# GuildOfWeavers/genSTARK

Measured on AMD Instinct MI355X. Metric: prove() ms + NTT GF(p) elements/sec, MiMC-128 2^20 steps, higher is better.
Workload: dtype u128; 1 GPU; MiMC-128 prove(), 2^20 steps, extensionFactor 16, exeQueryCount 48, friQueryCount 64, blake2s256; one independent proof per GPU; evaluation_domain=16777216, ntt_points_per_prove=17827072, ntt_transforms_per_prove=4, proof_bytes=371695

## Files before the change

genstark_amd/_abi.py:

```python
import ctypes as C
import os

_HERE = os.path.dirname(os.path.abspath(__file__))
HIP_LIB_PATH = os.path.join(_HERE, 'csrc', 'libgstark_hip.so')
MODULUS_128 = 2**128 - 9 * 2**32 + 1
MODULUS_64 = 2**64 - 21 * 2**30 + 1
MODULUS_32 = 2**32 - 3 * 2**25 + 1
MODULUS_17 = 96769
MODULUS_256 = 2**256 - 351 * 2**32 + 1
MODULUS_224 = 2**224 - 2**96 + 1
HIP_LIB_PATHS = {MODULUS_128: HIP_LIB_PATH, MODULUS_64: os.path.join(_HERE, 'csrc', 'libgstark_hip_q64.so'),
                 MODULUS_32: os.path.join(_HERE, 'csrc', 'libgstark_hip_q32.so'),
                 MODULUS_17: os.path.join(_HERE, 'csrc', 'libgstark_hip_q17.so'),
                 MODULUS_256: os.path.join(_HERE, 'csrc', 'libgstark_hip_p256.so'),
                 MODULUS_224: os.path.join(_HERE, 'csrc', 'libgstark_hip_p224.so')}
HIP_LIB_PATH_RUNTIME = os.path.join(_HERE, 'csrc', 'libgstark_hip_rt.so')

GS_OK = 0


class FriLayer(C.Structure):
    _fields_ = [('next', C.c_void_p), ('leaves', C.c_void_p), ('nodes', C.c_void_p), ('point_out', C.c_void_p), ('ticket', C.c_uint64)]

HASH_ALGS = {'sha256': 0, 'blake2s256': 1}
# ... 73 lines not shown
    'gs_small_interpolate': (_int, [_bytes, _bytes, _u32, _vp]),
    'gs_small_eval_poly': (_int, [_bytes, _u32, _bytes, _u32, _vp]),
    'gs_mimc_trace': (_int, [_vp, _bytes, _bytes, _u32, _u64, _vp]),
    'gs_mimc_constraints': (_int, [_vp, _vp, _u64, _u64, _vp, _u64, _vp]),
    'gs_mimc_composition': (_int, [_vp, _vp, _u64, _u64, _bytes, _vp, _u64, _bytes, _u64, _u64, _bytes, C.POINTER(_u64), _u32, _bytes, _vp]),
    'gs_pseudorandom_indexes': (_int, [_bytes, _u32, _u32, _u64, _u32, C.POINTER(_u64)]),
    'gs_air_trace_segments': (_int, [_vp, C.POINTER(_u32), _u32, C.POINTER(_u32), _u32, _bytes, _u32, _u32, _u32, _bytes, C.POINTER(_u32), _u32, _bytes, _u64, _u64, _vp]),
    'gs_air_trace': (_int, [_vp, C.POINTER(_u32), _u32, _bytes, _u32, _u32, _u32, _bytes, C.POINTER(_u32), _u32, _bytes, _u64, _vp]),
    'gs_air_constraints': (_int, [_vp, C.POINTER(_u32), _u32, _bytes, _u32, _u32, _u32, _u32, _vp, _u64, _u64, _vp,
                                  C.POINTER(_u64), _u32, _vp]),
    'gs_composition_tail': (_int, [_vp, _u64, _bytes, _vp, _vp, _u64, _bytes, _vp, _u32, _bytes, _u32, C.POINTER(_u64), C.POINTER(_u32), _u32, _bytes, _bytes,
                                   _vp, _u32, _bytes, _bytes, _vp, _u64, _vp, _vp]),
    'gs_composition_tail_coset': (_int, [_vp, _u64, _bytes, _bytes, _vp, _vp, _u64, _bytes, _vp, _u32, _bytes, _u32, C.POINTER(_u64), C.POINTER(_u32), _u32, _bytes,
                                         _bytes, _vp, _u32, _bytes, _bytes, _vp, _u64, _vp, _vp]),
    'gs_air_constraints_strided': (_int, [_vp, C.POINTER(_u32), _u32, _bytes, _u32, _u32, _u32, _u32, _vp, _u64, _u64, _u64, _u64, _vp,
                                          C.POINTER(_u64), _u32, _vp]),
}

EXPORTED_SYMBOLS = tuple(_SIGNATURES)

_OPTIONAL_SIGNATURES = {
    'gs_boundary_polys': (_int, [_vp, _bytes, _u64, _u64, C.POINTER(_u64), _bytes, C.POINTER(_u32), _u32, _u32, _vp, _vp]),
    'gs_boundary_schoolbook_log2': (_u32, [_u32]),
    'gs_eval_polys_at_points': (_int, [_vp, _vp, _u32, _u64, C.POINTER(_u64), _bytes, _u32, _vp]),
    'gs_eval_polys_at_points_segment': (_u32, []),
}
OPTIONAL_SYMBOLS = tuple(_OPTIONAL_SIGNATURES)

_HADES_SIGNATURES = {
    'gs_hades_create': (_int, [_vp, _u32, _u32, _u32, _u64, _bytes, _bytes, _pvp]),
    'gs_hades_destroy': (_int, [_vp, _vp]),
    'gs_hades_hash': (_int, [_vp, _vp, _vp, _u64, _u32, _u32, _vp]),
    'gs_hades_merkle': (_int, [_vp, _vp, _vp, _u64, _u32, _vp]),
    'gs_hades_merkle_paths': (_int, [_vp, _vp, _u64, _u32, C.POINTER(_u64), _u64, _vp]),
    'gs_hades_merkle_top': (_u32, []),
}
HADES_SYMBOLS = tuple(_HADES_SIGNATURES)

_RESCUE_SIGNATURES = {
    'gs_rescue_create': (_int, [_vp, _u32, _u32, _u64, _bytes, _bytes, _bytes, _pvp]),
    'gs_rescue_destroy': (_int, [_vp, _vp]),
    'gs_rescue_hash': (_int, [_vp, _vp, _vp, _u64, _u32, _u32, _u32, _u32, _vp]),
    'gs_rescue_merkle': (_int, [_vp, _vp, _vp, _u64, _vp]),
    'gs_rescue_spread_limit': (_u64, []),
}
RESCUE_SYMBOLS = tuple(_RESCUE_SIGNATURES)

_TREE_UPDATE_SIGNATURES = {
    'gs_hades_merkle_update': (_int, [_vp, _vp, _vp, _u64, _u32, C.POINTER(_u64), _vp, _u64, _vp, _vp]),
    'gs_rescue_merkle_update': (_int, [_vp, _vp, _vp, _u64, C.POINTER(_u64), _vp, _u64, _vp, _vp]),
}
TREE_UPDATE_SYMBOLS = tuple(_TREE_UPDATE_SIGNATURES)


class GstarkError(RuntimeError):
    pass


def load_library(path):
    if not os.path.exists(path):
        raise GstarkError(
            f'{path} not found: the HIP backend is not built (run `python -c "import __graft_entry__ as g; g.build()"`).'
            ' There is no CPU fallback.')
    lib = C.CDLL(path)
    for name, (res, args) in _SIGNATURES.items():
        fn = getattr(lib, name)
        fn.restype, fn.argtypes = res, args
    for name, (res, args) in (list(_OPTIONAL_SIGNATURES.items()) + list(_HADES_SIGNATURES.items()) + list(_RESCUE_SIGNATURES.items())
                              + list(_TREE_UPDATE_SIGNATURES.items())):
        fn = getattr(lib, name, None)
        if fn is not None:
            fn.restype, fn.argtypes = res, args
    return lib


class Backend:

    def __init__(self, device=0, stream=None, lib_path=None, allow_test_double=False, modulus=None):
        if lib_path is None:
            lib_path = HIP_LIB_PATH if modulus is None else HIP_LIB_PATHS.get(modulus, HIP_LIB_PATH_RUNTIME)
        self.lib = load_library(lib_path)
        self.element_size = self.lib.gs_element_size()
        if modulus is not None:
            if modulus < 3 or modulus >> (8 * self.element_size):
                raise GstarkError(f'a modulus of {modulus.bit_length()} bits does not fit {lib_path}')
            rc = self.lib.gs_set_modulus(modulus.to_bytes(self.element_size, 'little'), self.element_size)
            if rc != GS_OK:
                raise GstarkError(f'{lib_path} does not compute modulo {modulus} (gs_set_modulus: {rc}'
                                  + (': the runtime-modulus library serves ONE modulus per process, and it has been given another' if rc == -3 else '') + ')')
        buf = C.create_string_buffer(self.element_size)
        self.lib.gs_field_modulus(C.cast(buf, C.c_void_p))
        self.modulus = int.from_bytes(buf.raw, 'little')
        if modulus is not None and self.modulus != modulus:
            raise GstarkError(f'{lib_path} is built for the field of {self.modulus} elements, not {modulus}')
        if not self.modulus:
            raise GstarkError(f'{lib_path} takes its modulus at run time: pass modulus=')
        self.name = self.lib.gs_backend_name().decode()
        if self.name != 'hip-gfx950' and not allow_test_double:
            raise GstarkError(f'refusing backend {self.name!r}: the product path runs on hip-gfx950 only')
        if self.lib.gs_abi_version() != 1:
            raise GstarkError('gstark ABI version mismatch')
        ctx = C.c_void_p()
        rc = self.lib.gs_ctx_create(int(device), C.c_void_p(stream), C.byref(ctx))
        if rc != GS_OK or not ctx.value:
            raise GstarkError(f'gs_ctx_create(device={device}) failed with {rc}: no gfx950 device? (no CPU fallback)')
        self.ctx = ctx
        self.device = device
        self.stats = {}

    def jit(self, enable=True):
        self.call('gs_air_jit', 2 if enable == 'auto' else (1 if enable else 0))
        return self

    @property
    def jit_launches(self):
        return self.lib.gs_air_jit_launches(self.ctx)

    def traffic(self, on=None):
        if on is not None:
            self.call('gs_traffic_enable', 1 if on else 0)
            return self

# ... 66 lines not shown
```

genstark_amd/csrc/air_mimc.hip:

```cpp
#include "common.h"
#include "host_field.h"

__global__ void k_mimc_constraints(const fe *__restrict__ p, uint64_t nc, uint64_t shift, const fe *__restrict__ k, uint64_t klen,
                                   fe *__restrict__ out) {
    for (uint64_t j = blockIdx.x * (uint64_t)blockDim.x + threadIdx.x; j < nc; j += (uint64_t)gridDim.x * blockDim.x) {
        uint64_t jn = j + shift;
        if (jn >= nc) jn -= nc;
        fe x = p[j], nx = p[jn];
        fe x3 = fe_mul(fe_mul(x, x), x);
        out[j] = fe_sub(nx, fe_add(x3, k[j % klen]));
    }
}

#define GS_MIMC_COMP_MAX_PERIOD 32
#define GS_MIMC_COMP_MAX_ROOTS 4
struct MimcCompArgs {
    fe qz[GS_MIMC_COMP_MAX_PERIOD];
    fe bt[GS_MIMC_COMP_MAX_PERIOD];
    fe lt[GS_MIMC_COMP_MAX_PERIOD];
    fe ipoly[GS_MIMC_COMP_MAX_ROOTS];
    uint64_t root[GS_MIMC_COMP_MAX_ROOTS];
    fe x_last;
};
__global__ void k_mimc_composition(const fe *__restrict__ p, uint64_t n, uint64_t shift, const fe *__restrict__ k, uint64_t klen,
                                   const fe *__restrict__ tw_lo, const fe *__restrict__ tw_hi, int log_lo, int logn, const fe *__restrict__ u,
                                   MimcCompArgs a, uint32_t period, uint32_t nroots, int with_lc, fe *__restrict__ out) {
    __shared__ fe qz[GS_MIMC_COMP_MAX_PERIOD], bt[GS_MIMC_COMP_MAX_PERIOD], lt[GS_MIMC_COMP_MAX_PERIOD];
    if (threadIdx.x < period) { qz[threadIdx.x] = a.qz[threadIdx.x]; bt[threadIdx.x] = a.bt[threadIdx.x]; lt[threadIdx.x] = a.lt[threadIdx.x]; }
    __syncthreads();
    for (uint64_t i = blockIdx.x * (uint64_t)blockDim.x + threadIdx.x; i < n; i += (uint64_t)gridDim.x * blockDim.x) {
        fe x = tw_lo[i & ((1ull << log_lo) - 1)];
        if (logn > log_lo) x = fe_mul(x, tw_hi[i >> log_lo]);
        const fe pi = p[i], pn = p[(i + shift) & (n - 1)];
        const fe q = fe_sub(pn, fe_add(fe_mul(fe_mul(pi, pi), pi), k[i % klen]));
        const fe d = fe_mul(fe_mul(q, fe_sub(x, a.x_last)), qz[i & (period - 1)]);
        fe iv = a.ipoly[nroots - 1];
        for (int c = (int)nroots - 2; c >= 0; c--) iv = fe_add(fe_mul(iv, x), a.ipoly[c]);
        fe b = fe_mul(fe_sub(pi, iv), bt[i & (period - 1)]);
        for (uint32_t r = 0; r < nroots; r++) b = fe_mul(b, u[(i + n - a.root[r]) & (n - 1)]);
        fe r = fe_add(d, b);
        if (with_lc) r = fe_add(r, fe_mul(pi, lt[i & (period - 1)]));
        out[i] = r;
    }
}

#define GS_MIMC_CHUNK_BODY(STEP)                                                                                \
    for (uint64_t i = base; i < end; i++) {                                                                    \
        t[i] = hf_mimc_out(x);                                      \
        x = STEP(x, rc[ri]);                                   \
        if (++ri == nrc) ri = 0;                                                                               \
    }                                                                                                          \
    *ri_io = ri;                                                                                               \
    return x;
static hfe mimc_chunk_generic(hfe *t, hfe x, const hfe *rc, uint32_t nrc, uint32_t *ri_io, uint64_t base, uint64_t end) {
    uint32_t ri = *ri_io;
    GS_MIMC_CHUNK_BODY(hf_mimc_step_weak)
}
#if defined(__x86_64__) && !defined(__HIP_DEVICE_COMPILE__) && defined(GS_FIELD_128)
#define GS_MIMC_CHUNK_V3 1
__attribute__((target("arch=x86-64-v3,tune=znver5"))) static hfe mimc_chunk_v3(hfe *t, hfe x, const hfe *rc, uint32_t nrc, uint32_t *ri_io, uint64_t base,
                                                                               uint64_t end) {
    uint32_t ri = *ri_io;
    GS_MIMC_CHUNK_BODY(hf_cube_add_rows)
}
#endif
extern "C" {

int gs_mimc_trace(gs_ctx *c, const gs_elt *seed, const uint8_t *rc_host, uint32_t nrc, uint64_t steps, void *out) {
    if (!c || !seed || !rc_host || !out) return GS_ERR_ARG;
    if (!nrc || !steps) return gs_fail(c, GS_ERR_ARG, "mimc_trace: empty");
    std::vector<hfe> rc(nrc);
    for (uint32_t i = 0; i < nrc; i++) rc[i] = hf_load(rc_host + GS_ELT * i);
    int rcode = gs_trace_begin(c, steps * GS_ELT);
    if (rcode) return rcode;
    hfe *t = (hfe *)c->h_trace;
    hfe x = hf_load(seed);
    uint32_t ri = 0;
    const uint64_t CHUNK = 1ull << 16;
#ifdef GS_MIMC_CHUNK_V3
    static const bool v3 = __builtin_cpu_supports("avx2") && __builtin_cpu_supports("bmi2") && __builtin_cpu_supports("fma");
#else
    const bool v3 = false;
#endif
    for (uint64_t base = 0; base < steps; base += CHUNK) {
        const uint64_t end = base + CHUNK < steps ? base + CHUNK : steps;
#ifdef GS_MIMC_CHUNK_V3
        if (v3) x = mimc_chunk_v3(t, x, rc.data(), nrc, &ri, base, end);
        else
#endif
            x = mimc_chunk_generic(t, x, rc.data(), nrc, &ri, base, end);
        (void)v3;
        GS_HIP(c, hipMemcpyAsync((uint8_t *)out + base * GS_ELT, t + base, (end - base) * GS_ELT, hipMemcpyHostToDevice, c->stream));
    }
    return gs_trace_end(c);
}

int gs_mimc_constraints(gs_ctx *c, const void *p_comp, uint64_t nc, uint64_t shift, const void *k_table, uint64_t klen, void *out) {
    if (!c || !p_comp || !k_table || !out) return GS_ERR_ARG;
    if (!nc || !klen) return gs_fail(c, GS_ERR_ARG, "mimc_constraints: empty");
    hipLaunchKernelGGL(k_mimc_constraints, dim3(gs_grid(nc)), dim3(256), 0, c->stream, (const fe *)p_comp, nc, shift % nc,
                       (const fe *)k_table, klen, (fe *)out);
    GS_LAUNCH_CHECK(c);
    return GS_OK;
}

int gs_mimc_composition(gs_ctx *c, const void *p_eval, uint64_t n, uint64_t steps, const gs_elt *omega, const void *k_table, uint64_t klen,
                        const uint8_t *coeffs_host, uint64_t q_inc, uint64_t b_inc, const uint8_t *ipoly_host, const uint64_t *root_index_host,
                        uint32_t nroots, const uint8_t *lc_coeffs_host, void *out) {
    if (!c || !p_eval || !omega || !k_table || !coeffs_host || !ipoly_host || !root_index_host || !out) return GS_ERR_ARG;
    if (!gs_is_pow2(n) || !gs_is_pow2(steps) || steps > n || !klen) return gs_fail(c, GS_ERR_ARG, "mimc_composition: bad sizes");
    const uint64_t period = n / steps;
    if (period > GS_MIMC_COMP_MAX_PERIOD || nroots == 0 || nroots > GS_MIMC_COMP_MAX_ROOTS)
        return gs_fail(c, GS_ERR_UNSUPPORTED, "mimc_composition: n / steps <= %d and 1..%d assertions", GS_MIMC_COMP_MAX_PERIOD, GS_MIMC_COMP_MAX_ROOTS);
    if (q_inc % steps || b_inc % steps) return gs_fail(c, GS_ERR_ARG, "mimc_composition: degree increments must be multiples of the trace length");
    const fe w = fe_from_bytes(omega);
    const fe *lo, *hi, *u;
    int log_lo;
    int rc = gs_plan_pow_tables(c, w, n, &lo, &hi, &log_lo);
    if (!rc) rc = gs_plan_inverse_table(c, w, n, &u);
    if (rc) return rc;
    const fe d0 = fe_from_bytes(coeffs_host), d1 = fe_from_bytes(coeffs_host + GS_ELT), b0 = fe_from_bytes(coeffs_host + 2 * GS_ELT),
             b1 = fe_from_bytes(coeffs_host + 3 * GS_ELT);
    const fe l0 = lc_coeffs_host ? fe_from_bytes(lc_coeffs_host) : fe_zero(), l1 = lc_coeffs_host ? fe_from_bytes(lc_coeffs_host + GS_ELT) : fe_zero();
    MimcCompArgs a;
    uint64_t ksum = 0;
    for (uint32_t r = 0; r < GS_MIMC_COMP_MAX_ROOTS; r++) {
        a.root[r] = r < nroots ? root_index_host[r] & (n - 1) : 0;
        a.ipoly[r] = r < nroots ? fe_from_bytes(ipoly_host + GS_ELT * r) : fe_zero();
        if (r < nroots) ksum = (ksum + a.root[r]) & (n - 1);
    }
    const fe scale = gs_memo_pow(c, w, (n - ksum) & (n - 1));
    const std::vector<fe> &tab = gs_memo(c, gs_memo_key("mimc_comp").add(w).add(n).add(steps).add(q_inc).add(b_inc), [&](std::vector<fe> &t) {
        const fe g = fe_pow_u64(w, steps);
        const fe gq = fe_pow_u64(g, (q_inc / steps) % period), gb = fe_pow_u64(g, (b_inc / steps) % period);
        fe gj = fe_one(), gqj = fe_one(), gbj = fe_one();
        for (uint64_t j = 0; j < period; j++) {
            t.push_back(fe_inv(fe_sub(gj, fe_one())));
            t.push_back(gqj);
            t.push_back(gbj);
            gj = fe_mul(gj, g); gqj = fe_mul(gqj, gq); gbj = fe_mul(gbj, gb);
        }
        t.push_back(fe_pow_u64(w, (steps - 1) * period));
    });
    for (uint64_t j = 0; j < GS_MIMC_COMP_MAX_PERIOD; j++) {
        if (j < period) {
            a.qz[j] = fe_mul(fe_add(d0, fe_mul(d1, tab[3 * j + 1])), tab[3 * j]);
            a.bt[j] = fe_mul(fe_add(b0, fe_mul(b1, tab[3 * j + 2])), scale);
            a.lt[j] = fe_add(l0, fe_mul(l1, tab[3 * j + 2]));
        } else {
            a.qz[j] = a.bt[j] = a.lt[j] = fe_zero();
        }
    }
    a.x_last = tab[3 * period];
    gs_traffic(c, 2 * n * GS_ELT, n, "k_mimc_composition");
    hipLaunchKernelGGL(k_mimc_composition, dim3(gs_grid(n)), dim3(256), 0, c->stream, (const fe *)p_eval, n, period, (const fe *)k_table, klen, lo, hi,
                       log_lo, gs_log2(n), u, a, (uint32_t)period, nroots, lc_coeffs_host ? 1 : 0, (fe *)out);
    GS_LAUNCH_CHECK(c);
    return GS_OK;
}

}
```

genstark_amd/csrc/common.h:

```cpp
#pragma once
#include <hip/hip_runtime.h>
#include <stdint.h>
#include <stdio.h>
#include <stdarg.h>
#include <string.h>

#include <array>

#include <map>
#include <mutex>
#include <string>
#include <vector>

#include "../../include/gstark.h"
#if defined(GS_SMALL_Q)
#include "gf_small.h"
#elif defined(GS_WIDE_BITS)
#include "gf_wide.h"
#else
#include "gf128.h"
#define GS_FIELD_128 1
#endif

#if defined(GF_RUNTIME_MODULUS)
// ... 92 lines not shown
        if (c->scalar_memo.size() > 1024) c->scalar_memo.clear();
        it = c->scalar_memo.emplace(key.k, std::vector<fe>()).first;
        build(it->second);
    }
    return it->second;
}
static inline fe gs_memo_pow(gs_ctx *c, const fe &w, uint64_t e) {
    return gs_memo(c, gs_memo_key("pow").add(w).add(e), [&](std::vector<fe> &t) { t.push_back(fe_pow_u64(w, e)); })[0];
}

#define GS_HIP(c, call)                                                                              \
    do {                                                                                             \
        hipError_t e_ = (call);                                                                      \
        if (e_ != hipSuccess) return gs_fail((c), GS_ERR_DEVICE, "%s: %s", #call, hipGetErrorString(e_)); \
    } while (0)

#define GS_LAUNCH_CHECK(c) GS_HIP(c, hipGetLastError())

static inline bool gs_is_pow2(uint64_t x) { return x && !(x & (x - 1)); }
static inline int gs_log2(uint64_t x) { int l = 0; while ((1ull << l) < x) l++; return l; }

static inline fe fe_from_bytes(const uint8_t *b) { fe r; memcpy(&r, b, sizeof(fe)); return r; }
static inline void fe_to_bytes(uint8_t *b, const fe &v) { memcpy(b, &v, sizeof(fe)); }
static inline fe fe_from_u64(uint64_t v) { return fe_make((uint32_t)v, (uint32_t)(v >> 32), 0, 0); }

int gs_stage_reserve(gs_ctx *c, uint64_t bytes);
int gs_defer_flush(gs_ctx *c);
int gs_push_reserve(gs_ctx *c, uint64_t bytes, void **host);
int gs_push_commit(gs_ctx *c, void *dst, const void *host, uint64_t bytes);
int gs_push(gs_ctx *c, void *dst, const void *host_src, uint64_t bytes);
int gs_readback_reserve(gs_ctx *c, uint32_t bytes, void **slot_dev, unsigned long long **flag_dev, unsigned long long *value, uint64_t *ticket);
int gs_trace_begin(gs_ctx *c, uint64_t bytes);
int gs_trace_end(gs_ctx *c);
int gs_tmp_alloc(gs_ctx *c, uint64_t bytes, void **p);
void gs_tmp_free(gs_ctx *c, void *p);

static inline unsigned gs_grid(uint64_t work_items, unsigned block = 256, unsigned cap = 256 * 8) {
    uint64_t g = (work_items + block - 1) / block;
    if (g < 1) g = 1;
    if (g > cap) g = cap;
    return (unsigned)g;
}

int gs_jit_trace_segments(gs_ctx *c, const uint32_t *code, uint32_t ninstr, const uint32_t *icode, uint32_t init_ninstr, const uint8_t *consts_host,
                          uint32_t nconsts, uint32_t vm_regs, uint32_t registers, const uint64_t *soff, const uint64_t *slen, const uint8_t *statics_host,
                          uint32_t nstatic, const fe *dconst, const fe *dstat, const fe *drows, uint64_t segments, uint64_t seglen, fe *out);
int gs_jit_constraints(gs_ctx *c, const uint32_t *code, uint32_t ninstr, const uint8_t *consts_host, uint32_t nconsts, uint32_t vm_regs,
                       uint32_t registers, const uint64_t *soff, const uint64_t *slen, const fe *dconst, const fe *p, uint64_t nc, uint64_t shift,
                       const fe *statics, fe *out, uint64_t prow, uint64_t pstride);

void gs_plans_destroy(gs_ctx *c);
int gs_plan_pow_tables(gs_ctx *c, const fe &omega, uint64_t n, const fe **tw_lo, const fe **tw_hi, int *log_lo);
int gs_plan_inverse_table(gs_ctx *c, const fe &omega, uint64_t n, const fe **u);
int gs_plan_inverse_table_shifted(gs_ctx *c, const fe &omega, uint64_t n, const fe &shift, const fe **u);
```

genstark_amd/csrc/gf128.h:

```cpp
#pragma once
#include <stdint.h>

#if defined(__HIPCC__)
#define GF_HD __host__ __device__ __forceinline__
#else
#define GF_HD inline
#endif

struct alignas(16) fe {
    uint32_t w0, w1, w2, w3;
};

#define GF_P0 0x00000001u
#define GF_P1 0xFFFFFFF7u
#define GF_P2 0xFFFFFFFFu
#define GF_P3 0xFFFFFFFFu

GF_HD fe fe_make(uint32_t a, uint32_t b, uint32_t c, uint32_t d) { fe r; r.w0 = a; r.w1 = b; r.w2 = c; r.w3 = d; return r; }
GF_HD fe fe_zero() { return fe_make(0, 0, 0, 0); }
GF_HD fe fe_one() { return fe_make(1, 0, 0, 0); }
GF_HD bool fe_is_zero(const fe &a) { return (a.w0 | a.w1 | a.w2 | a.w3) == 0; }
GF_HD bool fe_eq(const fe &a, const fe &b) { return a.w0 == b.w0 && a.w1 == b.w1 && a.w2 == b.w2 && a.w3 == b.w3; }

GF_HD bool fe_ge_p(const fe &a) {
// ... 106 lines not shown
GF_HD uint32_t gf_fsh(uint32_t hi, uint32_t lo, int s) { return (hi << s) | (lo >> (32 - s)); }

GF_HD fe fe_reduce_wide(const uint32_t r[8]) {
    uint32_t c, b;
    uint64_t m = (uint64_t)r[4] * 9u;
    uint32_t a0 = (uint32_t)m;
    m = (uint64_t)r[5] * 9u + (m >> 32);
    uint32_t a1 = (uint32_t)m;
    m = (uint64_t)r[6] * 9u + (m >> 32);
    uint32_t a2 = (uint32_t)m;
    m = (uint64_t)r[7] * 9u + (m >> 32);
    uint32_t a3 = (uint32_t)m, a4 = (uint32_t)(m >> 32);
    uint32_t u1 = gf_addc(r[1], a0, 0u, c);
    uint32_t u2 = gf_addc(r[2], a1, c, c);
    uint32_t u3 = gf_addc(r[3], a2, c, c);
    uint32_t u4 = gf_addc(a3, 0u, c, c);
    uint32_t u5 = a4 + c;
    uint32_t v0 = gf_subc(r[0], r[4], 0u, b);
    uint32_t v1 = gf_subc(u1, r[5], b, b);
    uint32_t v2 = gf_subc(u2, r[6], b, b);
    uint32_t v3 = gf_subc(u3, r[7], b, b);
    uint32_t t0 = gf_subc(u4, 0u, b, b);
    uint32_t t1 = u5 - b;
    uint32_t g0 = gf_addc(t0 << 3, t0, 0u, c);
    uint32_t g1 = gf_fsh(t1, t0, 3) + t1 + c;
    uint32_t e0 = gf_subc(0u, t0, 0u, b);
    uint32_t e1 = gf_subc(g0, t1, b, b);
    uint32_t e2 = g1 - b;
    fe w;
    uint32_t k;
    w.w0 = gf_addc(v0, e0, 0u, c);
    w.w1 = gf_addc(v1, e1, c, c);
    w.w2 = gf_addc(v2, e2, c, c);
    w.w3 = gf_addc(v3, 0u, c, k);
    fe t;
    t.w0 = gf_addc(w.w0, 0xFFFFFFFFu, 0u, c);
    t.w1 = gf_addc(w.w1, 8u, c, c);
    t.w2 = gf_addc(w.w2, 0u, c, c);
    t.w3 = gf_addc(w.w3, 0u, c, c);
    bool sel = (k | c) != 0;
    fe o;
    o.w0 = sel ? t.w0 : w.w0;
    o.w1 = sel ? t.w1 : w.w1;
    o.w2 = sel ? t.w2 : w.w2;
    o.w3 = sel ? t.w3 : w.w3;
    return o;
}

GF_HD fe fe_mul(const fe &a, const fe &b) {
    uint32_t r[8];
    fe_mul_wide(a, b, r);
    return fe_reduce_wide(r);
}
GF_HD fe fe_sqr(const fe &a) { return fe_mul(a, a); }

GF_HD fe fe_pow(fe b, const fe &e) {
    fe r = fe_one();
    const uint32_t ev[4] = {e.w0, e.w1, e.w2, e.w3};
    for (int i = 0; i < 4; i++) {
        uint32_t w = ev[i];
        for (int k = 0; k < 32; k++) {
            if (w & 1u) r = fe_mul(r, b);
            b = fe_sqr(b);
            w >>= 1;
        }
    }
    return r;
}
GF_HD fe fe_pow_u64(fe b, uint64_t e) {
    if (!e) return fe_one();
    fe r = b;
    bool have = false;
    for (;;) {
        if (e & 1u) { r = have ? fe_mul(r, b) : b; have = true; }
        e >>= 1;
        if (!e) break;
        b = fe_sqr(b);
    }
    return r;
}

GF_HD fe fe_inv(const fe &a) {
    fe x1 = a;
    fe x2 = fe_mul(fe_sqr(x1), x1);
    fe x4 = fe_mul(fe_sqr(fe_sqr(x2)), x2);
    fe x8 = x4;
    for (int i = 0; i < 4; i++) x8 = fe_sqr(x8);
    x8 = fe_mul(x8, x4);
    fe x16 = x8;
    for (int i = 0; i < 8; i++) x16 = fe_sqr(x16);
    x16 = fe_mul(x16, x8);
    fe x32 = x16;
    for (int i = 0; i < 16; i++) x32 = fe_sqr(x32);
    x32 = fe_mul(x32, x16);
    fe x64 = x32;
    for (int i = 0; i < 32; i++) x64 = fe_sqr(x64);
    x64 = fe_mul(x64, x32);
    fe r = x64;
    fe x28 = x16;
    for (int i = 0; i < 8; i++) x28 = fe_sqr(x28);
    x28 = fe_mul(x28, x8);
    for (int i = 0; i < 4; i++) x28 = fe_sqr(x28);
    x28 = fe_mul(x28, x4);
    for (int i = 0; i < 28; i++) r = fe_sqr(r);
    r = fe_mul(r, x28);
    r = fe_sqr(r);
    r = fe_sqr(r); r = fe_mul(r, a);
// ... 7 lines not shown
```

genstark_amd/csrc/ntt.hip:

```cpp
#include "common.h"

#ifdef GS_FIELD_128
#include "gf128_lazy.h"
struct alignas(32) lz8 { int32_t l[8]; };
#endif

struct NttPlan {
    fe omega;
    uint64_t n = 0;
    int logn = 0, log_lo = 0;
    fe *tw_lo = nullptr;
    fe *tw_hi = nullptr;
    int npass = 0;
    int L[4] = {0, 0, 0, 0};
    fe *wR[4] = {nullptr, nullptr, nullptr, nullptr};
#ifndef GS_FIELD_128
    fe *twp[4] = {nullptr, nullptr, nullptr, nullptr};
#endif
    fe w16[8];
    fe *inv_table = nullptr;
    std::map<std::string, fe *> inv_table_shifted;
#ifdef GS_FIELD_128
    lzw *wtab = nullptr;
    lz8 *wRz[4] = {nullptr, nullptr, nullptr, nullptr};
    fe *twpR[4] = {nullptr, nullptr, nullptr, nullptr};
    fe *tw_loR = nullptr;
    lz8 *wRz_scaled = nullptr;
#endif
};

int gs_power_series_dev(gs_ctx *c, const fe &base, uint64_t n, fe *out);

__device__ __forceinline__ fe pow_lookup(const fe *__restrict__ tw_lo, const fe *__restrict__ tw_hi, int log_lo, int logn,
                                         uint64_t e) {
    fe x = tw_lo[e & ((1ull << log_lo) - 1)];
    if (logn > log_lo) x = fe_mul(x, tw_hi[e >> log_lo]);
    return x;
}

__host__ __device__ constexpr int brev(int i, int bits) {
    int r = 0;
    for (int b = 0; b < bits; b++) r |= ((i >> b) & 1) << (bits - 1 - b);
    return r;
}

#ifdef GS_FIELD_128
struct LzPassArgs {
    uint64_t n, in_len, in_stride, out_stride;
    int logn, logNs, logWj, log_lo;
    int scale;
    int exq0;
    int weak;
    const fe *tw_lo, *tw_hi, *twp;
    const fe *tw_loR;
    const lz8 *wR;
    const lzw *wtab;
};

#define LZ_FENCE() asm volatile("" ::: "memory")
#define LZ_PIN(x) asm volatile("" : "+v"((x).l[0]), "+v"((x).l[1]), "+v"((x).l[2]), "+v"((x).l[3]), "+v"((x).l[4]))
typedef const lzw *lzw_cptr;
__device__ __forceinline__ lzw lz_load_w(const lzw *p) {
    lzw W;
#if defined(__HIP_DEVICE_COMPILE__)
    const __attribute__((address_space(4))) int32_t *q = (const __attribute__((address_space(4))) int32_t *)(const int32_t *)p;
#pragma unroll
    for (int g = 0; g < 25; g += 8) {
#pragma unroll
        for (int e = g; e < g + 8 && e < 25; e++) W.w[e / 5][e % 5] = q[e];
        asm volatile("" ::: "memory");
    }
#else
    W = *p;
#endif
// ... 625 lines not shown
                    p->wRz[i] = (lz8 *)q;
                    hipLaunchKernelGGL(k_build_lz_table, dim3(gs_grid(R)), dim3(256), 0, c->stream, p->wR[i], p->wRz[i], R, lz_mont_r(), 1);
                }
#endif
            }
        }
    }
    c->plans[key] = p;
    *out = p;
    return GS_OK;
}

void gs_plans_destroy(gs_ctx *c) {
    for (auto &kv : c->plans) delete kv.second;
    c->plans.clear();
}

int gs_plan_pow_tables(gs_ctx *c, const fe &omega, uint64_t n, const fe **tw_lo, const fe **tw_hi, int *log_lo) {
    NttPlan *p;
    int rc = plan_get(c, omega, n, &p);
    if (rc) return rc;
    *tw_lo = p->tw_lo;
    *tw_hi = p->tw_hi;
    *log_lo = p->log_lo;
    return GS_OK;
}

__global__ void k_omega_minus_one(const fe *__restrict__ tw_lo, const fe *__restrict__ tw_hi, int log_lo, int logn, uint64_t n,
                                  fe shift, int has_shift, fe *__restrict__ out) {
    for (uint64_t i = blockIdx.x * (uint64_t)blockDim.x + threadIdx.x; i < n; i += (uint64_t)gridDim.x * blockDim.x) {
        fe x = pow_lookup(tw_lo, tw_hi, log_lo, logn, i);
        if (has_shift) x = fe_mul(x, shift);
        out[i] = fe_sub(x, fe_one());
    }
}

int gs_vec_inv_dev(gs_ctx *c, const fe *a, uint64_t n, fe *out);

int gs_plan_inverse_table(gs_ctx *c, const fe &omega, uint64_t n, const fe **u) {
    NttPlan *p;
    int rc = plan_get(c, omega, n, &p);
    if (rc) return rc;
    if (!p->inv_table) {
        void *q = nullptr, *t = nullptr;
        if ((rc = gs_alloc(c, n * GS_ELT, &q))) return rc;
        if ((rc = gs_tmp_alloc(c, n * GS_ELT, &t))) { gs_free(c, q); return rc; }
        hipLaunchKernelGGL(k_omega_minus_one, dim3(gs_grid(n)), dim3(256), 0, c->stream, p->tw_lo, p->tw_hi, p->log_lo, p->logn, n, fe_one(), 0, (fe *)t);
        rc = gs_vec_inv_dev(c, (const fe *)t, n, (fe *)q);
        gs_tmp_free(c, t);
        if (rc) { gs_free(c, q); return rc; }
        p->inv_table = (fe *)q;
    }
    *u = p->inv_table;
    return GS_OK;
}
int gs_plan_inverse_table_shifted(gs_ctx *c, const fe &omega, uint64_t n, const fe &shift, const fe **u) {
    if (fe_eq(shift, fe_one())) return gs_plan_inverse_table(c, omega, n, u);
    NttPlan *p;
    int rc = plan_get(c, omega, n, &p);
    if (rc) return rc;
    const std::string key = plan_key(shift, 0);
    auto it = p->inv_table_shifted.find(key);
    if (it == p->inv_table_shifted.end()) {
        void *q = nullptr, *t = nullptr;
        if ((rc = gs_alloc(c, n * GS_ELT, &q))) return rc;
        if ((rc = gs_tmp_alloc(c, n * GS_ELT, &t))) { gs_free(c, q); return rc; }
        hipLaunchKernelGGL(k_omega_minus_one, dim3(gs_grid(n)), dim3(256), 0, c->stream, p->tw_lo, p->tw_hi, p->log_lo, p->logn, n, shift, 1, (fe *)t);
        rc = gs_vec_inv_dev(c, (const fe *)t, n, (fe *)q);
        gs_tmp_free(c, t);
        if (rc) { gs_free(c, q); return rc; }
        it = p->inv_table_shifted.emplace(key, (fe *)q).first;
    }
    *u = it->second;
    return GS_OK;
}

#ifdef GS_FIELD_128
template <int LB>
static void launch_pass_lz(gs_ctx *c, const fe *in, fe *out, const LzPassArgs &a, uint32_t rows) {
    constexpr int RB = 1 << LB, R = 16 * RB;
    const int Wj = 1 << a.logWj;
    const uint64_t tiles = (a.n / R) / Wj;
    const bool first = a.logNs == 0;
    size_t lds = 0;
    if (RB > 1) lds = (size_t)5 * 4 * R * Wj;
    if (first) { const size_t tr = (size_t)Wj * (R + 1) * sizeof(fe); if (tr > lds) lds = tr; }
    gs_traffic(c, (uint64_t)rows * ((first ? a.in_len : a.n) + a.n) * GS_ELT, (uint64_t)rows * a.n, "k_ntt_pass_lz<%d, %d>", LB, first ? 0 : (a.twp ? 1 : 2));
    if (first) hipLaunchKernelGGL((k_ntt_pass_lz<LB, 0>), dim3((unsigned)tiles, rows), dim3(RB * Wj), lds, c->stream, in, out, a);
    else if (a.twp) hipLaunchKernelGGL((k_ntt_pass_lz<LB, 1>), dim3((unsigned)tiles, rows), dim3(RB * Wj), lds, c->stream, in, out, a);
    else hipLaunchKernelGGL((k_ntt_pass_lz<LB, 2>), dim3((unsigned)tiles, rows), dim3(RB * Wj), lds, c->stream, in, out, a);
}

template <int LB>
static void launch_pass_wave(gs_ctx *c, const fe *in, fe *out, const LzPassArgs &a, uint32_t rows) {
    constexpr int RB = 1 << LB, R = 16 * RB, Wj = 64 >> LB;
    const uint64_t tiles = (a.n / R) / Wj;
    gs_traffic(c, (uint64_t)rows * ((a.logNs == 0 ? a.in_len : a.n) + a.n) * GS_ELT, (uint64_t)rows * a.n, "k_ntt_wave<%d, %d>", LB, a.logNs == 0 ? 0 : (a.twp ? 1 : 2));
    if (a.logNs == 0) {
        if constexpr (LB == 4) hipLaunchKernelGGL((k_ntt_wave<4, 0>), dim3((unsigned)tiles, rows), dim3(64), 0, c->stream, in, out, a);
    } else if (a.twp) hipLaunchKernelGGL((k_ntt_wave<LB, 1>), dim3((unsigned)tiles, rows), dim3(64), 0, c->stream, in, out, a);
    else hipLaunchKernelGGL((k_ntt_wave<LB, 2>), dim3((unsigned)tiles, rows), dim3(64), 0, c->stream, in, out, a);
}
#else
template <int LB>
static void launch_pass(gs_ctx *c, const fe *in, fe *out, const PassArgs &a, uint32_t rows) {
    constexpr int RB = 1 << LB, R = 16 * RB;
// ... 157 lines not shown
```

genstark_amd/csrc/prover.cc:

```cpp
#include <dlfcn.h>
#include <stdarg.h>
#include <stdio.h>

#include <algorithm>
#include <map>
#include <chrono>
#include <deque>
#include <string>
#include <vector>

#include "../../include/gstark.h"
#include "../../include/gstark_prover.h"
#include "../../include/gstark_comm.h"
#include "../../include/gstark_boundary.h"
#if defined(GS_WIDE_BITS)
#include "gf_wide.h"
#endif
#include "host_field.h"
#include "host_poly.h"
#include "host_hash.h"

namespace {

#define GS_API_LIST(X)                                                                                                        \
    X(gs_alloc) X(gs_free) X(gs_upload) X(gs_download) X(gs_gather) X(gs_last_error) X(gs_power_series) X(gs_vec_add) X(gs_vec_mul) \
    X(gs_vec_sub_scalar) X(gs_vec_div) X(gs_combine_many) X(gs_combine_adjusted) X(gs_pluck) X(gs_transpose_vector) X(gs_sub_matrix_from_vectors)     \
    X(gs_eval_polys_at_roots) X(gs_interpolate_roots) X(gs_interpolate_quartic_domain) X(gs_eval_quartic_batch)                \
    X(gs_hash_merge_rows) X(gs_hash_digest_values) X(gs_merkle_build) X(gs_merkle_commit_rows) X(gs_merkle_prove_batch) X(gs_small_interpolate)          \
    X(gs_small_eval_poly) X(gs_pseudorandom_indexes) X(gs_mimc_trace) X(gs_mimc_constraints) X(gs_air_trace)                    \
    X(gs_air_trace_segments) X(gs_air_constraints) X(gs_air_constraints_strided) X(gs_composition_tail) X(gs_composition_tail_coset) X(gs_zero_poly_inverses) X(gs_div_by_domain_roots) X(gs_mimc_composition) X(gs_fri_fold) X(gs_fri_fold_seeded) X(gs_defer_begin) X(gs_defer_end) X(gs_readback_post) X(gs_readback_wait) X(gs_merkle_commit_rows_seed) X(gs_fri_fold_at) \
    X(gs_vec_mul_scalar) X(gs_copy) X(gs_gather_words) X(gs_transpose_records) X(gs_fri_fold_seeded_scaled) X(gs_fri_layers) X(gs_sync) X(gs_zero_poly_inverses_coset) X(gs_div_by_domain_roots_coset)
#define GS_API_OPTIONAL_LIST(X) X(gs_boundary_polys) X(gs_eval_polys_at_points)
struct Api {
#define X(name) decltype(&::name) name = nullptr;
    GS_API_LIST(X)
    GS_API_OPTIONAL_LIST(X)
#undef X
};
Api g_default_api;
bool g_bound = false;
thread_local const Api *g_api = &g_default_api;
#define A (*g_api)
struct UseApi {
    const Api *saved;
    explicit UseApi(const Api *a) : saved(g_api) { g_api = a; }
    ~UseApi() { g_api = saved; }
};

struct Fail {
    int code;
    std::string msg;
};
[[noreturn]] void fail(int code, const char *fmt, ...) {
    char buf[512];
    va_list ap;
    va_start(ap, fmt);
    vsnprintf(buf, sizeof buf, fmt, ap);
    va_end(ap);
    throw Fail{code, buf};
}

typedef hfe F;
const uint64_t ELEM = HF_ELT;
const uint64_t DIGEST = 32, MAX_ARRAY = 256;
const uint64_t WORD = 16, EW = ELEM / WORD;
static_assert(ELEM <= GS_PROVER_ELT_MAX, "element wider than the job's scalar fields");
typedef std::vector<uint8_t> Bytes;

struct Ctx {
    gs_ctx *c;
    void check(int rc, const char *what) {
        if (rc) fail(rc, "%s: %s", what, c ? A.gs_last_error(c) : "error");
    }
};

struct Buf {
    Ctx *x = nullptr;
    void *p = nullptr;
    Buf() {}
    Buf(Ctx &cx, uint64_t bytes) : x(&cx) { cx.check(A.gs_alloc(cx.c, bytes ? bytes : 16, &p), "gs_alloc"); }
    Buf(const Buf &) = delete;
    Buf &operator=(const Buf &) = delete;
    Buf(Buf &&o) noexcept : x(o.x), p(o.p) { o.p = nullptr; }
    Buf &operator=(Buf &&o) noexcept {
        if (this != &o) { release(); x = o.x; p = o.p; o.p = nullptr; }
// ... 849 lines not shown
    for (uint64_t l = len; l > 256; l /= 4) {
        const uint64_t rows = l / 4;
        folds.emplace_back();
        Fold &f = folds.back();
        f.next = Buf(x, rows * ELEM);
        f.cTree.n = rows / 4;
        f.cTree.leaves = Buf(x, rows / 4 * DIGEST);
        f.cTree.nodes = Buf(x, rows / 4 * DIGEST);
        if (rows > 256) f.cTree.point = Buf(x, ELEM);
        f.cTree.root.resize(DIGEST);
    }
    if (folds.empty()) return folds;
    std::vector<gs_fri_layer> outs(folds.size());
    for (size_t d = 0; d < folds.size(); d++) outs[d] = gs_fri_layer{folds[d].next.p, folds[d].cTree.leaves.p, folds[d].cTree.nodes.p, folds[d].cTree.point.p, 0};
    x.check(A.gs_fri_layers(x.c, (gs_hash_alg)alg, enc(omega), N, step, column, len, point, (uint32_t)outs.size(), outs.data()), "gs_fri_layers");
    for (size_t d = 0; d < folds.size(); d++) folds[d].cTree.ticket = outs[d].ticket;
    return folds;
}

}

static void prove_impl(Ctx &x, const gs_prover_job &job, Bytes &out) {
    PhaseClock clock;
    const gs_prover_air &air = job.air;
    const uint64_t T = job.steps, E = job.extension_factor, N = T * E;
    const uint32_t R = air.registers;
    const int alg = job.hash_alg;
    check_job(job);
    const Shapes input_shapes = checked_job_shapes(job);
    check_extension_factor(job);
    const F omega = domain_root(job, N);
    Plan plan = make_plan(job, T, E, omega, false);
    const uint64_t Nc = plan.Nc, combination_degree = plan.combination_degree, b_inc = plan.b_inc;
    const F comp_rou = hf_pow(omega, (hfe)(N / Nc)), exec_rou = hf_pow(omega, (hfe)E);
    const Coset domain{N, omega, 1, E, true};


    uint32_t assertions_on_r0 = 0;
    for (uint32_t i = 0; i < job.nassertions; i++) assertions_on_r0 += job.assertions[i].reg == 0;
    const bool fused = air.kind == 0 && E <= 32 && air.nconstraints == 1 && assertions_on_r0 == job.nassertions && job.nassertions <= 4;
    const bool tail = !fused && tail_fits(job, R + air.nsecret);
    const bool tail_makes_z = tail && domain.unit <= 32;
    uint32_t most_assertions = 0;
    for (auto &r : plan.regs) most_assertions = std::max(most_assertions, (uint32_t)r.steps.size());
    const uint32_t DEVICE_BOUNDARY_ABOVE = 128;
    const bool device_boundary = !fused && !tail && most_assertions > DEVICE_BOUNDARY_ABOVE && A.gs_boundary_polys && !g_host_boundary && plan.regs.size() <= 64 &&
                                 most_assertions <= T && T <= (1ull << 28);
    if (!device_boundary) plan.fill_xs();
    Buf zInverses;
    if (!fused && !tail_makes_z) zInverses = zero_poly_inverses(x, plan, domain);
    Buf psbPowers;
    const bool lc_folds = fused && R + air.nsecret == 1;
    if (b_inc > 0 && !lc_folds && !tail) psbPowers = coset_powers(x, domain, b_inc);

    Buf kN;
    uint64_t klen_n = 0;
    if (air.kind == 0) {
        klen_n = air.k_len * (N / Nc);
        Buf kPoly(x, air.k_len * ELEM);
        kN = Buf(x, klen_n * ELEM);
        x.check(counted_interpolate_roots(x.c, air.k_table, 1, enc(hf_pow(omega, (hfe)(N / air.k_len))), air.k_len, kPoly.p), "gs_interpolate_roots(K)");
        x.check(counted_eval_polys_at_roots(x.c, kPoly.p, 1, air.k_len, enc(hf_pow(omega, (hfe)(N / klen_n))), klen_n, kN.p), "gs_eval_polys_at_roots(K)");
    }

    clock.mark("context + trace-independent work issued");
    clock.readme(x, "Set up evaluation context");
    Buf trace(x, (uint64_t)R * T * ELEM);
    launch_trace(x, job, air.first_rows, air.segments, trace.p);
    check_assertion_ranges(job);
    std::vector<uint64_t> asserted_at;
    for (uint32_t i = 0; i < job.nassertions; i++) asserted_at.push_back((uint64_t)job.assertions[i].reg * T + job.assertions[i].step);

    clock.mark("execution trace (host recurrence)");
    clock.readme(x, "Generated execution trace");
    Buf pPolys(x, (uint64_t)R * T * ELEM), pEval(x, (uint64_t)R * N * ELEM);
    x.check(counted_interpolate_roots(x.c, trace.p, R, enc(exec_rou), T, pPolys.p), "gs_interpolate_roots(trace)");
    clock.readme(x, "Computed execution trace polynomials P(x)");
    x.check(counted_eval_polys_at_roots(x.c, pPolys.p, R, T, enc(omega), N, pEval.p), "gs_eval_polys_at_roots(P)");
    clock.readme(x, "Low-degree extended P(x) polynomials over evaluation domain");
    std::vector<const void *> pRows(R);
    for (uint32_t r = 0; r < R; r++) pRows[r] = pEval.at((uint64_t)r * N * ELEM);
    std::vector<const void *> eVectors(pRows);
    for (uint32_t i = 0; i < air.nsecret; i++) eVectors.push_back(air.secret_traces[i]);
    const uint32_t V = (uint32_t)eVectors.size();

    Tree eTree = commit_rows(x, alg, eVectors.data(), V, N, false);

    clock.mark("P(x), extension, evaluation tree issued");
    clock.readme(x, "Serialized evaluations of P(x) and S(x) polynomials + Built evaluation merkle tree (one fused call)");
    const uint32_t dcount = plan.dcount, bcoef = plan.bcoef;
    std::vector<F> coefficients;
    auto read_evaluation_root = [&] {
        Bytes got(asserted_at.size() * ELEM);
        const uint64_t one = 1;
        DeferWindow win(x);
        x.check(A.gs_gather(x.c, trace.p, ELEM, asserted_at.data(), asserted_at.size(), got.data()), "gs_gather(asserted cells)");
        x.check(A.gs_gather(x.c, eTree.nodes.p, DIGEST, &one, 1, eTree.root.data()), "gs_gather(root)");
        win.end();
        check_asserted_cells(job, [&](uint32_t i) { return got.data() + i * ELEM; });
        trace.release();
        coefficients = plan.coefficients(eTree.root, V);
    };

    Buf cEval(x, N * ELEM);
    bool lc_fused = false;
    if (fused) {
// ... 138 lines not shown
```

Measured before the change: 1.608 billion elements/s.

## Process MiMC composition in quarter-domain quads with precomputed boundary inverse product

The MiMC composition kernel now has each thread handle four points i + s*n/4 that share one twiddle computation, using x*iota and -x symmetry to derive the other x values and the boundary interpolant cheaply. The per-point product of several boundary inverse factors is replaced by a single lookup into a cached product table, built once per root set and prepared early in the prover. A dedicated squaring routine replaces the general multiply for the cube. This removes redundant twiddle loads and multiplies per point at the cost of an extra n-sized table and more registers per thread.

New measurement: 1.605 billion elements/s. No clear change (-0.2%).

```diff
diff --git a/genstark_amd/_abi.py b/genstark_amd/_abi.py
--- a/genstark_amd/_abi.py
+++ b/genstark_amd/_abi.py
@@ -149,6 +149,12 @@
 }
 TREE_UPDATE_SYMBOLS = tuple(_TREE_UPDATE_SIGNATURES)
 
+_MIMC_SIGNATURES = {
+    'gs_mimc_composition_prepare': (_int, [_vp, _bytes, _u64, C.POINTER(_u64), _u32]),
+    'gs_mimc_composition_quads': (_int, [_vp, _bytes, _u64, _u64]),
+}
+MIMC_SYMBOLS = tuple(_MIMC_SIGNATURES)
+
 
 class GstarkError(RuntimeError):
     pass
@@ -164,7 +170,7 @@
         fn = getattr(lib, name)
         fn.restype, fn.argtypes = res, args
     for name, (res, args) in (list(_OPTIONAL_SIGNATURES.items()) + list(_HADES_SIGNATURES.items()) + list(_RESCUE_SIGNATURES.items())
-                              + list(_TREE_UPDATE_SIGNATURES.items())):
+                              + list(_TREE_UPDATE_SIGNATURES.items()) + list(_MIMC_SIGNATURES.items())):
         fn = getattr(lib, name, None)
         if fn is not None:
             fn.restype, fn.argtypes = res, args
diff --git a/genstark_amd/csrc/air_mimc.hip b/genstark_amd/csrc/air_mimc.hip
--- a/genstark_amd/csrc/air_mimc.hip
+++ b/genstark_amd/csrc/air_mimc.hip
@@ -1,5 +1,6 @@
 #include "common.h"
 #include "host_field.h"
+#include "../../include/gstark_mimc.h"
 
 __global__ void k_mimc_constraints(const fe *__restrict__ p, uint64_t nc, uint64_t shift, const fe *__restrict__ k, uint64_t klen,
                                    fe *__restrict__ out) {
@@ -21,10 +22,49 @@
     fe ipoly[GS_MIMC_COMP_MAX_ROOTS];
     uint64_t root[GS_MIMC_COMP_MAX_ROOTS];
     fe x_last;
+    fe iota, neg_x_last;
 };
-__global__ void k_mimc_composition(const fe *__restrict__ p, uint64_t n, uint64_t shift, const fe *__restrict__ k, uint64_t klen,
-                                   const fe *__restrict__ tw_lo, const fe *__restrict__ tw_hi, int log_lo, int logn, const fe *__restrict__ u,
-                                   MimcCompArgs a, uint32_t period, uint32_t nroots, int with_lc, fe *__restrict__ out) {
+__global__ void k_mimc_composition(const fe *__restrict__ p, uint64_t n, uint64_t shift, const fe *__restrict__ k, uint64_t klen, int k_shared,
+                                   const fe *__restrict__ tw_lo, const fe *__restrict__ tw_hi, int log_lo, int logn, const fe *__restrict__ U,
+                                   uint64_t uoff, MimcCompArgs a, uint32_t period, uint32_t nroots, int with_lc, fe *__restrict__ out) {
+    __shared__ fe qz[GS_MIMC_COMP_MAX_PERIOD], bt[GS_MIMC_COMP_MAX_PERIOD], lt[GS_MIMC_COMP_MAX_PERIOD];
+    if (threadIdx.x < period) { qz[threadIdx.x] = a.qz[threadIdx.x]; bt[threadIdx.x] = a.bt[threadIdx.x]; lt[threadIdx.x] = a.lt[threadIdx.x]; }
+    __syncthreads();
+    const uint64_t nq = n >> 2;
+    for (uint64_t i = blockIdx.x * (uint64_t)blockDim.x + threadIdx.x; i < nq; i += (uint64_t)gridDim.x * blockDim.x) {
+        fe x0 = tw_lo[i & ((1ull << log_lo) - 1)];
+        if (logn > log_lo) x0 = fe_mul(x0, tw_hi[i >> log_lo]);
+        const fe x1 = fe_mul(x0, a.iota);
+        const uint32_t j = (uint32_t)i & (period - 1);
+        const fe qzj = qz[j], btj = bt[j], ltj = lt[j];
+        fe m0 = fe_zero(), m1 = fe_zero();
+        if (nroots == 2) { m0 = fe_mul(a.ipoly[1], x0); m1 = fe_mul(a.ipoly[1], x1); }
+        const uint64_t kq = i % klen;
+#pragma unroll
+        for (int s = 0; s < 4; s++) {
+            const uint64_t is = i + s * nq;
+            const fe xs = (s & 1) ? x1 : x0, ms = (s & 1) ? m1 : m0;
+            const fe pi = p[is], pn = p[(is + shift) & (n - 1)];
+            const fe ks = k[k_shared ? kq : is % klen];
+            const fe q = fe_sub(pn, fe_add(fe_mul(fe_sqr(pi), pi), ks));
+            const fe d = fe_mul(fe_mul(q, (s & 2) ? fe_sub(a.neg_x_last, xs) : fe_sub(xs, a.x_last)), qzj);
+            fe iv;
+            if (nroots <= 2) iv = (s & 2) ? fe_sub(a.ipoly[0], ms) : fe_add(a.ipoly[0], ms);
+            else {
+                const fe x = (s & 2) ? fe_sub(fe_zero(), xs) : xs;
+                iv = a.ipoly[nroots - 1];
+                for (int c = (int)nroots - 2; c >= 0; c--) iv = fe_add(fe_mul(iv, x), a.ipoly[c]);
+            }
+            const fe b = fe_mul(fe_mul(fe_sub(pi, iv), btj), U[(is + n - uoff) & (n - 1)]);
+            fe r = fe_add(d, b);
+            if (with_lc) r = fe_add(r, fe_mul(pi, ltj));
+            out[is] = r;
+        }
+    }
+}
+__global__ void k_mimc_composition_points(const fe *__restrict__ p, uint64_t n, uint64_t shift, const fe *__restrict__ k, uint64_t klen,
+                                          const fe *__restrict__ tw_lo, const fe *__restrict__ tw_hi, int log_lo, int logn, const fe *__restrict__ U,
+                                          uint64_t uoff, MimcCompArgs a, uint32_t period, uint32_t nroots, int with_lc, fe *__restrict__ out) {
     __shared__ fe qz[GS_MIMC_COMP_MAX_PERIOD], bt[GS_MIMC_COMP_MAX_PERIOD], lt[GS_MIMC_COMP_MAX_PERIOD];
     if (threadIdx.x < period) { qz[threadIdx.x] = a.qz[threadIdx.x]; bt[threadIdx.x] = a.bt[threadIdx.x]; lt[threadIdx.x] = a.lt[threadIdx.x]; }
     __syncthreads();
@@ -32,12 +72,11 @@
         fe x = tw_lo[i & ((1ull << log_lo) - 1)];
         if (logn > log_lo) x = fe_mul(x, tw_hi[i >> log_lo]);
         const fe pi = p[i], pn = p[(i + shift) & (n - 1)];
-        const fe q = fe_sub(pn, fe_add(fe_mul(fe_mul(pi, pi), pi), k[i % klen]));
+        const fe q = fe_sub(pn, fe_add(fe_mul(fe_sqr(pi), pi), k[i % klen]));
         const fe d = fe_mul(fe_mul(q, fe_sub(x, a.x_last)), qz[i & (period - 1)]);
         fe iv = a.ipoly[nroots - 1];
         for (int c = (int)nroots - 2; c >= 0; c--) iv = fe_add(fe_mul(iv, x), a.ipoly[c]);
-        fe b = fe_mul(fe_sub(pi, iv), bt[i & (period - 1)]);
-        for (uint32_t r = 0; r < nroots; r++) b = fe_mul(b, u[(i + n - a.root[r]) & (n - 1)]);
+        const fe b = fe_mul(fe_mul(fe_sub(pi, iv), bt[i & (period - 1)]), U[(i + n - uoff) & (n - 1)]);
         fe r = fe_add(d, b);
         if (with_lc) r = fe_add(r, fe_mul(pi, lt[i & (period - 1)]));
         out[i] = r;
@@ -64,6 +103,13 @@
     GS_MIMC_CHUNK_BODY(hf_cube_add_rows)
 }
 #endif
+static int mimc_boundary_inverses(gs_ctx *c, const fe &w, uint64_t n, const uint64_t *root_index, uint32_t nroots, const fe **U) {
+    return nroots == 1 ? gs_plan_inverse_table(c, w, n, U) : gs_plan_inverse_product_table(c, w, n, root_index, nroots, U);
+}
+static bool mimc_composition_takes_quads(gs_ctx *c, const fe &w, uint64_t n, uint64_t steps) {
+    return steps >= 4 && fe_eq(gs_memo_pow(c, w, n / 2), fe_neg(fe_one()));
+}
+
 extern "C" {
 
 int gs_mimc_trace(gs_ctx *c, const gs_elt *seed, const uint8_t *rc_host, uint32_t nrc, uint64_t steps, void *out) {
@@ -114,10 +160,10 @@
         return gs_fail(c, GS_ERR_UNSUPPORTED, "mimc_composition: n / steps <= %d and 1..%d assertions", GS_MIMC_COMP_MAX_PERIOD, GS_MIMC_COMP_MAX_ROOTS);
     if (q_inc % steps || b_inc % steps) return gs_fail(c, GS_ERR_ARG, "mimc_composition: degree increments must be multiples of the trace length");
     const fe w = fe_from_bytes(omega);
-    const fe *lo, *hi, *u;
+    const fe *lo, *hi, *U;
     int log_lo;
     int rc = gs_plan_pow_tables(c, w, n, &lo, &hi, &log_lo);
-    if (!rc) rc = gs_plan_inverse_table(c, w, n, &u);
+    if (!rc) rc = mimc_boundary_inverses(c, w, n, root_index_host, nroots, &U);
     if (rc) return rc;
     const fe d0 = fe_from_bytes(coeffs_host), d1 = fe_from_bytes(coeffs_host + GS_ELT), b0 = fe_from_bytes(coeffs_host + 2 * GS_ELT),
              b1 = fe_from_bytes(coeffs_host + 3 * GS_ELT);
@@ -152,11 +198,33 @@
         }
     }
     a.x_last = tab[3 * period];
+    a.iota = gs_memo_pow(c, w, n / 4);
+    a.neg_x_last = fe_neg(a.x_last);
+    const uint64_t uoff = nroots == 1 ? a.root[0] : 0;
     gs_traffic(c, 2 * n * GS_ELT, n, "k_mimc_composition");
-    hipLaunchKernelGGL(k_mimc_composition, dim3(gs_grid(n)), dim3(256), 0, c->stream, (const fe *)p_eval, n, period, (const fe *)k_table, klen, lo, hi,
-                       log_lo, gs_log2(n), u, a, (uint32_t)period, nroots, lc_coeffs_host ? 1 : 0, (fe *)out);
+    if (mimc_composition_takes_quads(c, w, n, steps))
+        hipLaunchKernelGGL(k_mimc_composition, dim3(gs_grid(n / 4)), dim3(256), 0, c->stream, (const fe *)p_eval, n, period, (const fe *)k_table, klen,
+                           (n / 4) % klen == 0 ? 1 : 0, lo, hi, log_lo, gs_log2(n), U, uoff, a, (uint32_t)period, nroots, lc_coeffs_host ? 1 : 0, (fe *)out);
+    else
+        hipLaunchKernelGGL(k_mimc_composition_points, dim3(gs_grid(n)), dim3(256), 0, c->stream, (const fe *)p_eval, n, period, (const fe *)k_table, klen,
+                           lo, hi, log_lo, gs_log2(n), U, uoff, a, (uint32_t)period, nroots, lc_coeffs_host ? 1 : 0, (fe *)out);
     GS_LAUNCH_CHECK(c);
     return GS_OK;
 }
 
-}
+int gs_mimc_composition_prepare(gs_ctx *c, const gs_elt *omega, uint64_t n, const uint64_t *root_index_host, uint32_t nroots) {
+    if (!c || !omega || !root_index_host) return GS_ERR_ARG;
+    if (!gs_is_pow2(n) || nroots == 0 || nroots > GS_MIMC_COMP_MAX_ROOTS) return gs_fail(c, GS_ERR_ARG, "mimc_composition_prepare: n a power of two, 1..%d assertions", GS_MIMC_COMP_MAX_ROOTS);
+    const fe w = fe_from_bytes(omega);
+    const fe *lo, *hi, *U;
+    int log_lo;
+    const int rc = gs_plan_pow_tables(c, w, n, &lo, &hi, &log_lo);
+    return rc ? rc : mimc_boundary_inverses(c, w, n, root_index_host, nroots, &U);
+}
+
+int gs_mimc_composition_quads(gs_ctx *c, const gs_elt *omega, uint64_t n, uint64_t steps) {
+    if (!c || !omega || !gs_is_pow2(n) || !gs_is_pow2(steps) || steps > n) return 0;
+    return mimc_composition_takes_quads(c, fe_from_bytes(omega), n, steps) ? 1 : 0;
+}
+
+}
diff --git a/genstark_amd/csrc/common.h b/genstark_amd/csrc/common.h
--- a/genstark_amd/csrc/common.h
+++ b/genstark_amd/csrc/common.h
@@ -168,4 +168,5 @@
 void gs_plans_destroy(gs_ctx *c);
 int gs_plan_pow_tables(gs_ctx *c, const fe &omega, uint64_t n, const fe **tw_lo, const fe **tw_hi, int *log_lo);
 int gs_plan_inverse_table(gs_ctx *c, const fe &omega, uint64_t n, const fe **u);
+int gs_plan_inverse_product_table(gs_ctx *c, const fe &omega, uint64_t n, const uint64_t *root_index, uint32_t nroots, const fe **U);
 int gs_plan_inverse_table_shifted(gs_ctx *c, const fe &omega, uint64_t n, const fe &shift, const fe **u);
diff --git a/genstark_amd/csrc/gf128.h b/genstark_amd/csrc/gf128.h
--- a/genstark_amd/csrc/gf128.h
+++ b/genstark_amd/csrc/gf128.h
@@ -182,7 +182,35 @@
     fe_mul_wide(a, b, r);
     return fe_reduce_wide(r);
 }
-GF_HD fe fe_sqr(const fe &a) { return fe_mul(a, a); }
+GF_HD void fe_sqr_wide(const fe &a, uint32_t r[8]) {
+    uint64_t t = (uint64_t)a.w0 * a.w1;
+    uint32_t c1 = (uint32_t)t;
+    t = (uint64_t)a.w0 * a.w2 + (t >> 32);
+    uint32_t c2 = (uint32_t)t;
+    t = (uint64_t)a.w0 * a.w3 + (t >> 32);
+    uint32_t c3 = (uint32_t)t, c4 = (uint32_t)(t >> 32);
+    t = (uint64_t)a.w1 * a.w2 + c3;
+    c3 = (uint32_t)t;
+    t = (uint64_t)a.w1 * a.w3 + (t >> 32) + c4;
+    c4 = (uint32_t)t;
+    t = (uint64_t)a.w2 * a.w3 + (t >> 32);
+    uint32_t c5 = (uint32_t)t, c6 = (uint32_t)(t >> 32);
+    const uint64_t s0 = (uint64_t)a.w0 * a.w0, s1 = (uint64_t)a.w1 * a.w1, s2 = (uint64_t)a.w2 * a.w2, s3 = (uint64_t)a.w3 * a.w3;
+    uint32_t c;
+    r[0] = (uint32_t)s0;
+    r[1] = gf_addc((uint32_t)(s0 >> 32), c1 << 1, 0u, c);
+    r[2] = gf_addc((uint32_t)s1, gf_fsh(c2, c1, 1), c, c);
+    r[3] = gf_addc((uint32_t)(s1 >> 32), gf_fsh(c3, c2, 1), c, c);
+    r[4] = gf_addc((uint32_t)s2, gf_fsh(c4, c3, 1), c, c);
+    r[5] = gf_addc((uint32_t)(s2 >> 32), gf_fsh(c5, c4, 1), c, c);
+    r[6] = gf_addc((uint32_t)s3, gf_fsh(c6, c5, 1), c, c);
+    r[7] = (uint32_t)(s3 >> 32) + (c6 >> 31) + c;
+}
+GF_HD fe fe_sqr(const fe &a) {
+    uint32_t r[8];
+    fe_sqr_wide(a, r);
+    return fe_reduce_wide(r);
+}
 
 GF_HD fe fe_pow(fe b, const fe &e) {
     fe r = fe_one();
diff --git a/genstark_amd/csrc/ntt.hip b/genstark_amd/csrc/ntt.hip
--- a/genstark_amd/csrc/ntt.hip
+++ b/genstark_amd/csrc/ntt.hip
@@ -20,6 +20,8 @@
     fe w16[8];
     fe *inv_table = nullptr;
     std::map<std::string, fe *> inv_table_shifted;
+    fe *inv_product = nullptr;
+    std::string inv_product_roots;
 #ifdef GS_FIELD_128
     lzw *wtab = nullptr;
     lz8 *wRz[4] = {nullptr, nullptr, nullptr, nullptr};
@@ -751,6 +753,40 @@
         p->inv_table = (fe *)q;
     }
     *u = p->inv_table;
+    return GS_OK;
+}
+__global__ void k_inverse_product_table(const fe *__restrict__ u, uint64_t n, uint64_t r0, uint64_t r1, uint64_t r2, uint64_t r3, uint32_t nroots,
+                                        fe *__restrict__ out) {
+    for (uint64_t i = blockIdx.x * (uint64_t)blockDim.x + threadIdx.x; i < n; i += (uint64_t)gridDim.x * blockDim.x) {
+        fe v = fe_mul(u[(i + n - r0) & (n - 1)], u[(i + n - r1) & (n - 1)]);
+        if (nroots > 2) v = fe_mul(v, u[(i + n - r2) & (n - 1)]);
+        if (nroots > 3) v = fe_mul(v, u[(i + n - r3) & (n - 1)]);
+        out[i] = v;
+    }
+}
+int gs_plan_inverse_product_table(gs_ctx *c, const fe &omega, uint64_t n, const uint64_t *root_index, uint32_t nroots, const fe **U) {
+    if (nroots < 2 || nroots > 4 || !gs_is_pow2(n)) return gs_fail(c, GS_ERR_ARG, "inverse product table: 2..4 roots, n a power of two");
+    const fe *u;
+    int rc = gs_plan_inverse_table(c, omega, n, &u);
+    if (rc) return rc;
+    NttPlan *p;
+    if ((rc = plan_get(c, omega, n, &p))) return rc;
+    uint64_t r[4] = {0, 0, 0, 0};
+    for (uint32_t a = 0; a < nroots; a++) r[a] = root_index[a] & (n - 1);
+    const std::string key((const char *)r, nroots * sizeof(uint64_t));
+    if (!p->inv_product || p->inv_product_roots != key) {
+        if (!p->inv_product) {
+            void *q = nullptr;
+            if ((rc = gs_alloc(c, n * GS_ELT, &q))) return rc;
+            p->inv_product = (fe *)q;
+        }
+        p->inv_product_roots.clear();
+        hipLaunchKernelGGL(k_inverse_product_table, dim3(gs_grid(n)), dim3(256), 0, c->stream, u, n, r[0], r[1], r[2], r[3], nroots, p->inv_product);
+        GS_LAUNCH_CHECK(c);
+        gs_traffic(c, (uint64_t)(nroots + 1) * n * GS_ELT, n, "k_inverse_product_table");
+        p->inv_product_roots = key;
+    }
+    *U = p->inv_product;
     return GS_OK;
 }
 int gs_plan_inverse_table_shifted(gs_ctx *c, const fe &omega, uint64_t n, const fe &shift, const fe **u) {
diff --git a/genstark_amd/csrc/prover.cc b/genstark_amd/csrc/prover.cc
--- a/genstark_amd/csrc/prover.cc
+++ b/genstark_amd/csrc/prover.cc
@@ -13,6 +13,7 @@
 #include "../../include/gstark_prover.h"
 #include "../../include/gstark_comm.h"
 #include "../../include/gstark_boundary.h"
+#include "../../include/gstark_mimc.h"
 #if defined(GS_WIDE_BITS)
 #include "gf_wide.h"
 #endif
@@ -30,7 +31,7 @@
     X(gs_small_eval_poly) X(gs_pseudorandom_indexes) X(gs_mimc_trace) X(gs_mimc_constraints) X(gs_air_trace)                    \
     X(gs_air_trace_segments) X(gs_air_constraints) X(gs_air_constraints_strided) X(gs_composition_tail) X(gs_composition_tail_coset) X(gs_zero_poly_inverses) X(gs_div_by_domain_roots) X(gs_mimc_composition) X(gs_fri_fold) X(gs_fri_fold_seeded) X(gs_defer_begin) X(gs_defer_end) X(gs_readback_post) X(gs_readback_wait) X(gs_merkle_commit_rows_seed) X(gs_fri_fold_at) \
     X(gs_vec_mul_scalar) X(gs_copy) X(gs_gather_words) X(gs_transpose_records) X(gs_fri_fold_seeded_scaled) X(gs_fri_layers) X(gs_sync) X(gs_zero_poly_inverses_coset) X(gs_div_by_domain_roots_coset)
-#define GS_API_OPTIONAL_LIST(X) X(gs_boundary_polys) X(gs_eval_polys_at_points)
+#define GS_API_OPTIONAL_LIST(X) X(gs_boundary_polys) X(gs_eval_polys_at_points) X(gs_mimc_composition_prepare)
 struct Api {
 #define X(name) decltype(&::name) name = nullptr;
     GS_API_LIST(X)
@@ -986,6 +987,10 @@
     Buf psbPowers;
     const bool lc_folds = fused && R + air.nsecret == 1;
     if (b_inc > 0 && !lc_folds && !tail) psbPowers = coset_powers(x, domain, b_inc);
+    if (fused && A.gs_mimc_composition_prepare) {
+        const Plan::Boundary at = plan.boundary(E, false);
+        x.check(A.gs_mimc_composition_prepare(x.c, enc(omega), N, at.at.data(), at.per_row[0]), "gs_mimc_composition_prepare");
+    }
 
     Buf kN;
     uint64_t klen_n = 0;
diff --git a/include/gstark_mimc.h b/include/gstark_mimc.h
--- /dev/null
+++ b/include/gstark_mimc.h
@@ -0,0 +1,17 @@
+#ifndef GSTARK_MIMC_H
+#define GSTARK_MIMC_H
+
+#include "gstark.h"
+
+#ifdef __cplusplus
+extern "C" {
+#endif
+
+int gs_mimc_composition_prepare(gs_ctx *ctx, const gs_elt *omega, uint64_t n, const uint64_t *root_index_host, uint32_t nroots);
+
+int gs_mimc_composition_quads(gs_ctx *ctx, const gs_elt *omega, uint64_t n, uint64_t steps);
+
+#ifdef __cplusplus
+}
+#endif
+#endif
```
